# lfalive/fast-genomic-data-processing

Measured on AMD Instinct MI355X. Metric: PairHMM GCUPS, higher is better.
Workload: dtype f32

## Files before the change

### fast-genomic-data-processing_amd/csrc/mgx_pairhmm.hip

```cpp
#include <hip/hip_runtime.h>

#include <algorithm>
#include <atomic>
#include <cerrno>
#include <cmath>
#include <cstdio>
#include <cstdlib>
#include <cstring>
#include <chrono>
#include <memory>
#include <mutex>
#include <new>
#include <thread>
#include <string>
#include <vector>

#include "../../include/mgx_pairhmm.h"
#include "../../include/mgx_realign.h"
#include "mgx_hip_util.h"
#include "mgx_realign_internal.h"
#include "mgx_tables.h"
#include "pairhmm_pack.h"
#include "pairhmm_plan.h"
#include "pairhmm_wire.h"
// ... 463 lines not shown
int ensure_strip_scratch(mgx_pairhmm* c, size_t bytes) {
    if (bytes <= c->strip_cap) return 0;
    HIP_TRY(hipStreamSynchronize(c->compute));
    (void)hipFree(c->d_strip); c->d_strip = nullptr; c->strip_cap = 0;
    HIP_TRY(hipMalloc(&c->d_strip, bytes));
    c->strip_cap = bytes;
    return 0;
}

int pick_event_set(Run& r) {
    mgx_pairhmm_batch* b = r.b;
    if (!r.timing) return 0;
    if (b->ev.empty()) {
        const size_t per = b->bins.size() * 4;
        b->ev_sets = (uint32_t)std::max<size_t>(1, std::min<size_t>(kMaxEventSets, 1024 / per));
        b->ev.resize(per * b->ev_sets);
        for (auto& e : b->ev) HIP_TRY(hipEventCreate(&e));
    }
    r.ev = b->ev.data() + (size_t)(b->runs_timed % b->ev_sets) * b->bins.size() * 4;
    return 0;
}

int begin_run(Run& r) {
    mgx_pairhmm* c = r.c; mgx_pairhmm_batch* b = r.b;
    if (b->uploaded) HIP_TRY(hipStreamWaitEvent(r.s, b->uploaded, 0));
    HIP_TRY(hipMemsetAsync(b->counters(), 0, kCounters * sizeof(uint32_t), r.s));
    HIP_TRY(hipMemsetAsync(b->dev(b->lay.o_used), 0, b->n_pairs, r.s));
    KernelArgs& base = r.base;
    base.jobs = b->dev<Job>(b->lay.jobs);
    base.bases = b->dev(b->lay.seq[kSeqBases]); base.qual = b->dev(b->lay.seq[kSeqQual]); base.ins = b->dev(b->lay.seq[kSeqIns]); base.del = b->dev(b->lay.seq[kSeqDel]);
    base.gcp = b->dev(b->lay.seq[kSeqGcp]); base.hap_bases = b->dev(b->lay.seq[kSeqHap]);
    base.out_log10 = b->dev<double>(b->lay.o_out); base.used_f64 = b->dev(b->lay.o_used);
    base.nhap_list = b->dev<uint32_t>(b->lay.nlist); base.nhap_count = b->counters() + kNhapCount;
    base.log10_initial_f = c->log10_initial_f;
    base.log10_initial_d = c->log10_initial_d;
    return 0;
}

int launch_f64(const Run& r, KernelArgs a, int Gd, int RPLd, uint32_t grid, uint32_t block, uint32_t lds) {
    const mgx_pairhmm* c = r.c;
    a.ph2pr = c->d_ph2pr_d; a.mm = c->d_mm_d; a.ph2pr_div3 = c->d_div3_d; a.gap_ratio = c->d_ratio_d;
    a.rerun_list = r.b->rerun_list() + r.b->n_pairs; a.rerun_count = r.b->counters() + kExactCount;
    KernelFn f = a.strip_scratch ? (KernelFn)pairhmm_fwd_strip<double> : pick_kernel<double>(Gd, RPLd);
    if (!f) { set_error("no fp64 kernel for G=%d RPL=%d", Gd, RPLd); return -ENOSYS; }
    hipLaunchKernelGGL(f, dim3(grid), dim3(block), lds, r.s, a);
    return 0;
}

int launch_multi(Run& r, int gset, const MultiSet& ms) {
    mgx_pairhmm* c = r.c; mgx_pairhmm_batch* b = r.b;
    const std::vector<size_t>& set = ms.members;
    MultiArgs m{};
    m.a = r.base;
    m.a.rerun_list = b->rerun_list(); m.a.rerun_count = b->counters() + kSharedCount;
    m.a.job_list = nullptr; m.a.n_dyn = nullptr;
    m.a.ph2pr = c->d_ph2pr_f; m.a.mm = c->d_mm_f; m.a.ph2pr_div3 = c->d_div3_f; m.a.gap_ratio = c->d_ratio_f;
    m.n_bins = (uint32_t)set.size();
    size_t book = set[0];
    uint64_t cells = 0, bytes = 0;
    for (size_t q = 0; q < set.size(); ++q) {
        const Bin& bn = b->bins[set[q]];
        m.job_first[q] = bn.job_begin; m.job_count[q] = bn.job_count; m.lds_stride[q] = bn.lds_stride;
        m.G[q] = (uint8_t)bn.G; m.RPL[q] = (uint8_t)bn.RPL; m.bin[q] = (uint8_t)set[q];
        if (bn.cells > b->bins[book].cells) book = set[q];
        cells += bn.cells; bytes += bn.alg_bytes;
        r.in_multi[set[q]] = 1;
// ... 144 lines not shown

int mgx_pairhmm_batch_read_inputs(mgx_pairhmm_t* c, mgx_pairhmm_batch_t* b, uint8_t* bases, uint8_t* qual, uint8_t* ins,
                                  uint8_t* del, uint8_t* gcp, uint8_t* hap) {
    if (!c || !b) { set_error("ctx/batch is NULL"); return -EINVAL; }
    if ((b->lay.read_bytes && (!bases || !qual || !ins || !del || !gcp)) || (b->lay.hap_bytes && !hap)) { set_error("NULL argument"); return -EINVAL; }
    HIP_TRY(hipSetDevice(c->device));
    if (b->n_pairs == 0) return 0;
    if (b->uploaded) HIP_TRY(hipEventSynchronize(b->uploaded));
    uint8_t* const host[kSeqArrays] = {bases, qual, ins, del, gcp, hap};
    for (int k = 0; k < kSeqArrays; ++k) {
        const uint64_t len = k == kSeqHap ? b->lay.hap_bytes : b->lay.read_bytes;
        if (len) HIP_TRY(hipMemcpy(host[k], b->dev(b->lay.seq[k]), len, hipMemcpyDeviceToHost));
    }
    return 0;
}

int mgx_pairhmm_sync(mgx_pairhmm_t* c) {
    if (!c) { set_error("ctx is NULL"); return -EINVAL; }
    HIP_TRY(hipSetDevice(c->device));
    HIP_TRY(hipStreamSynchronize(c->compute));
    return 0;
}

int mgx_pairhmm_batch_stats(mgx_pairhmm_t* c, mgx_pairhmm_batch_t* b, mgx_pairhmm_stats_t* out) {
    if (!c || !b || !out) { set_error("NULL argument"); return -EINVAL; }
    HIP_TRY(hipSetDevice(c->device));
    HIP_TRY(hipStreamSynchronize(c->compute));
    mgx_pairhmm_stats_t st = b->stats;
    const bool force_f64 = (c->flags & MGX_PAIRHMM_FORCE_DOUBLE) != 0;
    st.n_launches_f32 = force_f64 ? 0 : (uint32_t)b->bins.size();
    st.n_launches_f64 = (uint32_t)b->bins.size();
    st.n_rerun_f64 = 0;
    st.n_nhap_f32 = 0;
    if (b->ran && b->n_pairs) {
        std::vector<uint32_t> cnt(kCounters);
        HIP_TRY(hipMemcpy(cnt.data(), b->counters(), kCounters * sizeof(uint32_t), hipMemcpyDeviceToHost));
        for (size_t k = 0; k < b->bins.size(); ++k) st.n_nhap_f32 += cnt[kNhapCount + k];
        for (size_t k = 0; k < b->bins.size(); ++k) st.n_rerun_f64 += force_f64 ? b->bins[k].job_count : cnt[k];
        if (!force_f64) st.n_rerun_f64 += cnt[kSharedCount];
        st.n_exact = cnt[kExactCount];
    }
    st.ms_f32 = st.ms_f64 = st.ms_f32_dominant = 0;
    st.dominant_cells = st.dominant_alg_bytes = 0;
    st.dominant_kernel[0] = 0;
    st.n_runs_timed = 0;
    if ((c->flags & MGX_PAIRHMM_TIMING) && b->ran && !b->ev.empty() && b->runs_timed) {
        const uint32_t n_sets = std::min(b->runs_timed, b->ev_sets);
        const bool acct = b->acct_cells.size() == b->bins.size();
        auto cells_of = [&](size_t k) { return acct ? b->acct_cells[k] : b->bins[k].cells; };
        size_t dom = 0;
        for (size_t k = 0; k < b->bins.size(); ++k) if (cells_of(k) >= cells_of(dom)) dom = k;
        double f32 = 0, f64 = 0, domms = 0;
        for (uint32_t q = 0; q < n_sets; ++q) {
            const uint32_t set = (b->runs_timed - 1 - q) % b->ev_sets;
            hipEvent_t* ev = b->ev.data() + (size_t)set * b->bins.size() * 4;
            for (size_t k = 0; k < b->bins.size(); ++k) {
                float ms = 0;
                if (!force_f64) {
                    HIP_TRY(hipEventElapsedTime(&ms, ev[4 * k + 0], ev[4 * k + 1]));
                    f32 += ms;
                    if (k == dom) domms += ms;
                }
                float ms2 = 0;
                HIP_TRY(hipEventElapsedTime(&ms2, ev[4 * k + 2], ev[4 * k + 3]));
                f64 += ms2;
            }
        }
        st.n_runs_timed = n_sets;
        st.ms_f32 = (float)(f32 / n_sets); st.ms_f64 = (float)(f64 / n_sets);
        if (!force_f64) {
// ... 404 lines not shown
```

### fast-genomic-data-processing_amd/csrc/pairhmm_kernels.hip.inc

```

#include <type_traits>

#include "best_allele_rule.h"
#include "pairhmm_plan.h"

namespace {

using namespace mgx_hmm_plan;

struct KernelArgs {
    const Job* jobs;
    const uint32_t* job_list;
    const uint32_t* n_dyn;
    uint32_t n_static;
    uint32_t job_first;
    const uint8_t* bases;
    const uint8_t* qual;
    const uint8_t* ins;
    const uint8_t* del;
    const uint8_t* gcp;
    const uint8_t* hap_bases;
    const void* ph2pr;
    const void* mm;
    const void* ph2pr_div3;
    const void* gap_ratio;
    double* out_log10;
    uint8_t* used_f64;
    uint32_t* rerun_list;
    uint32_t* rerun_count;
    uint32_t* nhap_list;
    uint32_t* nhap_count;
    uint32_t lds_stride;
    void* strip_scratch;
    uint32_t strip_stride;
    float log10_initial_f;
    double log10_initial_d;
};

constexpr double kExactBelow = 1e-280;
constexpr int kCodeN = 4;
constexpr int kCodePad = 7;

__device__ __forceinline__ int base_code(int b) {
    int c = 0;
    c = (b == 'C') ? 1 : c;
    c = (b == 'T') ? 2 : c;
    c = (b == 'G') ? 3 : c;
    c = (b == 'N') ? kCodeN : c;
    return c;
}

__device__ __forceinline__ uint32_t base_code4(uint32_t w) {
    const uint32_t sel = (w >> 1) & 0x07070707u;
    const uint32_t code = __builtin_amdgcn_perm(0x04000000u, 0x03020100u, sel);
    const uint32_t want = __builtin_amdgcn_perm(0x4E000000u, 0x47544341u, sel);
    const uint32_t diff = want ^ w;
    const uint32_t nz = (((diff & 0x7F7F7F7Fu) + 0x7F7F7F7Fu) | diff) & 0x80808080u;
    const uint32_t ok = ((nz ^ 0x80808080u) >> 7) * 0xFFu;
    return code & ok;
}

template <int G> constexpr int lane_stride() { return G < 16 ? 16 / G : 1; }

template <int G>
// ... 7 lines not shown
__device__ __forceinline__ float shr1(float old, float v) {
    return __builtin_bit_cast(float, dpp_shr1<G>(__builtin_bit_cast(int, old), __builtin_bit_cast(int, v)));
}
template <int G>
__device__ __forceinline__ double shr1(double old, double v) {
    long long o = __builtin_bit_cast(long long, old), x = __builtin_bit_cast(long long, v);
    unsigned lo = (unsigned)dpp_shr1<G>((int)(unsigned)o, (int)(unsigned)x);
    unsigned hi = (unsigned)dpp_shr1<G>((int)(unsigned)(o >> 32), (int)(unsigned)(x >> 32));
    return __builtin_bit_cast(double, ((long long)hi << 32) | (long long)lo);
}

template <int G, typename T>
__device__ __forceinline__ T shr1_down(T v) {
    const int lane = (int)(threadIdx.x & 63);
    constexpr int S = lane_stride<G>();
    const int j = G < 16 ? (lane & 15) / S : lane % G;
    const int src = (j == G - 1) ? lane : lane + S;
    return __shfl(v, src, 64);
}

__device__ __forceinline__ float fma_(float a, float b, float c) { return __builtin_fmaf(a, b, c); }
__device__ __forceinline__ double fma_(double a, double b, double c) { return __builtin_fma(a, b, c); }

template <typename T> struct Prec;
template <> struct Prec<float> {
    static __device__ __forceinline__ float initial() { return 0x1p120f; }
};
template <> struct Prec<double> {
    static __device__ __forceinline__ double initial() { return 0x1p1020; }
};

template <int RPL, int CODES> constexpr int etab_bytes_per_wave() { return ((RPL + 1) / 2) * CODES * 64 * 8; }

template <typename T, int G, int RPL, bool STRIP = false, bool EXACT = false, int CODES = kMaxCodes>
__device__ __forceinline__ void pairhmm_body(const KernelArgs& a, uint8_t* smem, const uint32_t block, const uint32_t n_blocks) {
    constexpr int GPW = 64 / G;
    constexpr bool kETab = (sizeof(T) == 4);
    constexpr int kNumCodes = CODES;
    static_assert(CODES == 4 || CODES == kMaxCodes, "four or five code columns");
    static_assert(kETab || CODES == kMaxCodes, "fp64 has no table: the N code is compared");
    constexpr bool kSix = (sizeof(T) == 4) && !EXACT;
    constexpr int RP2 = (RPL + 1) / 2;
    constexpr int S = lane_stride<G>();
    const int gpb = (int)blockDim.x / G;
    const int tid = (int)threadIdx.x;
    const int lane = tid & 63;
    const int wave = tid >> 6;
    const int j = G < 16 ? (lane & 15) / S : lane % G;
    const int grp = wave * GPW + (G < 16 ? (lane >> 4) * S + (lane & 15) % S : lane / G);
    const int n_waves = (int)blockDim.x >> 6;
    uint8_t* etab = smem + (kETab ? (size_t)wave * etab_bytes_per_wave<RPL, CODES>() : 0);
    uint8_t* hapbuf = smem + (kETab ? (size_t)n_waves * etab_bytes_per_wave<RPL, CODES>() : 0) +
                      (size_t)grp * a.lds_stride;
    const T* __restrict__ ph2pr = (const T*)a.ph2pr;
    const T* __restrict__ mm = (const T*)a.mm;
    const T* __restrict__ ph2pr_div3 = (const T*)a.ph2pr_div3;
    const T* __restrict__ gap_ratio = (const T*)a.gap_ratio;
    const uint32_t n_jobs = a.n_dyn ? *a.n_dyn : a.n_static;

    for (uint32_t base = block * (uint32_t)gpb; base < n_jobs; base += n_blocks * (uint32_t)gpb) {
        const uint32_t slot = base + (uint32_t)grp;
        const bool live = slot < n_jobs;
        uint32_t job_idx = 0;
        Job job;
        job.read_off = 0; job.hap_off = 0; job.R = 0; job.H = 0; job.pair = 0; job.pad_ = 0;
        if (live) {
            job_idx = a.job_list ? a.job_list[slot] : a.job_first + slot;
            job = a.jobs[job_idx];
        }
        const int R = (int)job.R, H = (int)job.H;
        constexpr int kStripRows = G * RPL;
        const int n_strips = STRIP ? (R > kStripRows ? (R + kStripRows - 1) / kStripRows : 1) : 1;
        const int first_rows = R - (n_strips - 1) * kStripRows;

        __syncthreads();
        bool hap_n = false;
        {
            const uint8_t* hp = a.hap_bases + job.hap_off;
            const int n_words = (int)a.lds_stride >> 2;
            uint32_t* hb32 = reinterpret_cast<uint32_t*>(hapbuf);
            for (int w = j; w < n_words; w += G) {
                const int c0 = 4 * w - G;
                uint32_t packed;
                if (live && c0 >= 0 && c0 + 4 <= H) {
                    uint32_t raw;
                    __builtin_memcpy(&raw, hp + c0, 4);
                    packed = base_code4(raw);
                } else {
                    packed = 0;
#pragma unroll
                    for (int t = 0; t < 4; ++t) {
                        const int c = c0 + t;
                        const int code = (live && c >= 0 && c < H) ? base_code(hp[c]) : (kNumCodes > 4 ? kCodeN : 0);
                        packed |= (uint32_t)code << (8 * t);
                    }
                }
                if constexpr (kETab && kNumCodes == 4) {
                    const uint32_t x = packed ^ (0x01010101u * (uint32_t)kCodeN);
                    hap_n |= ((x - 0x01010101u) & ~x & 0x80808080u) != 0;
                    packed &= 0x03030303u;
                }
                hb32[w] = packed;
            }
        }
        bool group_hap_n = false;
        if constexpr (kETab && kNumCodes == 4) {
            uint64_t gmask;
            if constexpr (G == 64) gmask = ~0ull;
            else if constexpr (G == 16) gmask = 0xFFFFull << (lane & 48);
            else gmask = (uint64_t)((G == 8 ? 0x5555u : 0x1111u) << ((lane & 15) % S)) << (lane & 48);
            group_hap_n = (__ballot((int)hap_n) & gmask) != 0;
        }

        T sumM = 0, sumX = 0;
        bool zero_gap = false;
        if constexpr (STRIP) {
            for (int rr = lane; rr < R; rr += 64) zero_gap |= (a.gcp[job.read_off + (uint64_t)rr] & 127) == 0;
        }
        int nl = 0;
        T* const bnd = STRIP ? reinterpret_cast<T*>(a.strip_scratch) + (size_t)block * 6u * a.strip_stride : nullptr;
      for (int strip = 0; strip < n_strips; ++strip) {
        const int rows_here = (STRIP && strip > 0) ? kStripRows : first_rows;
        const int row_base = (STRIP && strip > 0) ? first_rows + (strip - 1) * kStripRows : 0;
        const bool last_strip = strip == n_strips - 1;
        nl = (rows_here + RPL - 1) / RPL;
        const int top_clones = nl * RPL - rows_here;
        volatile T* const bcur = STRIP ? bnd + (size_t)(strip & 1) * 3u * a.strip_stride : nullptr;
        const volatile T* const bprev = STRIP ? bnd + (size_t)((strip & 1) ^ 1) * 3u * a.strip_stride : nullptr;
        if (STRIP && strip > 0) __syncthreads();

        T k0[RPL], k1[RPL], k2[RPL], k3[RPL], k4[RPL], eM[RPL], eX[RPL];
        int rb[RPL];
        T pm[RPL], px[RPL], py[RPL];
        bool clone[RPL];
        T ratio[RPL];
        const T init_y = Prec<T>::initial() / (T)(H > 0 ? H : 1);
#pragma unroll
        for (int s = 0; s < RPL; ++s) {
            const int rho = j * RPL + s - top_clones;
            k0[s] = 0; k1[s] = 0; k2[s] = 0; k3[s] = 0; k4[s] = 0; eM[s] = 0; eX[s] = 0;
            rb[s] = 0; pm[s] = 0; px[s] = 0; py[s] = 0; clone[s] = false; ratio[s] = 0;
            if (live && j < nl) {
                if (rho < 0) {
                    clone[s] = true;
                    k3[s] = 1;
                    py[s] = init_y;
                } else {
                    const uint64_t o = job.read_off + (uint64_t)(row_base + rho);
                    const int qi = a.ins[o] & 127, qd = a.del[o] & 127, qc = a.gcp[o] & 127;
                    const int qq = a.qual[o] & 127;
                    const int mn = qi <= qd ? qi : qd, mx = qi <= qd ? qd : qi;
                    k0[s] = mm[((mx * (mx + 1)) >> 1) + mn];
                    k3[s] = ph2pr[qc];
                    k1[s] = (T)1.0 - ph2pr[qc];
                    k2[s] = ph2pr[qi];
                    k4[s] = ph2pr[qd];
                    zero_gap |= (qc == 0);
                    const T distm = ph2pr[qq];
                    eM[s] = (T)1.0 - distm;
                    const int code = base_code(a.bases[o]);
                    eX[s] = (code == kCodeN) ? eM[s] : ph2pr_div3[qq];
                    ratio[s] = gap_ratio[qc];
                    rb[s] = code;
                }
            }
        }
        if constexpr (kETab) {
            float* et = reinterpret_cast<float*>(etab) + lane * 2;
#pragma unroll
            for (int s = 0; s < RPL; ++s)
#pragma unroll
                for (int code = 0; code < kNumCodes; ++code)
                    et[((s >> 1) * kNumCodes + code) * 128 + (s & 1)] =
                        (code == rb[s] || code == kCodeN) ? eM[s] : eX[s];
        }
        __syncthreads();

        const bool swept = live && !group_hap_n;
        const int nsteps_g = swept ? (H + nl - 1) : 0;
        int nmax = nsteps_g, nmin = swept ? nsteps_g : 0x7fffffff;
        if constexpr (GPW > 1) {
#pragma unroll
            for (int off = 1; off < 64; off <<= 1) {
                if (off >= S && off < (G < 16 ? 16 : G)) continue;
                const int o1 = __shfl_xor(nmax, off, 64), o2 = __shfl_xor(nmin, off, 64);
                nmax = o1 > nmax ? o1 : nmax;
                nmin = o2 < nmin ? o2 : nmin;
            }
        }
        nmax = __builtin_amdgcn_readfirstlane(nmax);
        nmin = __builtin_amdgcn_readfirstlane(nmin);
        if (nmin > nmax) nmin = nmax;

        const uint8_t* hp_lane = hapbuf + (G - j);
        const uint8_t* et_lane = etab + lane * 8;

        auto load_e = [&](int h, T (&dst)[RPL]) {
            if constexpr (kETab) {
                const uint8_t* p = et_lane + (h << 9);
#pragma unroll
                for (int s2 = 0; s2 < RP2; ++s2) {
                    const float2 v = *reinterpret_cast<const float2*>(p + s2 * kNumCodes * 512);
                    dst[2 * s2] = v.x;
                    if (2 * s2 + 1 < RPL) dst[2 * s2 + 1] = v.y;
                }
            } else {
                const bool hN = (h == kCodeN);
#pragma unroll
                for (int s = 0; s < RPL; ++s) dst[s] = ((h == rb[s]) | hN) ? eM[s] : eX[s];
            }
        };

        const bool use_plain = EXACT || __any((int)zero_gap) != 0;
        constexpr int kPlain = 0, kScaled = 1, kSixOp = 2;

        auto sweep = [&](auto form_tag) {
            constexpr int FORM = decltype(form_tag)::value;
            constexpr bool SC = FORM == kScaled;
            constexpr bool SIX = FORM == kSixOp;
            T y_above = init_y;
            if constexpr (SC || SIX) {
                T g_own[RPL], g_below[RPL];
#pragma unroll
                for (int s = 0; s < RPL; ++s) g_own[s] = k1[s];
                T g_next_lane = shr1_down<G>(g_own[0]);
#pragma unroll
                for (int s = 0; s < RPL; ++s) g_below[s] = (s + 1 < RPL) ? g_own[s + 1] : g_next_lane;
                if (j == nl - 1) {
                    g_below[RPL - 1] = (T)1.0;
                    if constexpr (STRIP) { if (!last_strip) g_below[RPL - 1] = (T)1.0 - ph2pr[a.gcp[job.read_off + (uint64_t)(row_base + rows_here)] & 127]; }
                }
                T my_above[RPL];
                if constexpr (SIX) {
                    T my_own[RPL];
#pragma unroll
                    for (int s = 0; s < RPL; ++s) my_own[s] = clone[s] ? (T)1.0 : k4[s];
                    T my_top = (T)1.0;
                    if constexpr (STRIP) {
                        if (strip > 0) my_top = ph2pr[a.del[job.read_off + (uint64_t)(row_base - 1)] & 127];
                    }
                    my_above[0] = shr1<G>(my_top, my_own[RPL - 1]);
#pragma unroll
                    for (int s = 1; s < RPL; ++s) my_above[s] = my_own[s - 1];
                }
#pragma unroll
                for (int s = 0; s < RPL; ++s) {
                    if (clone[s]) {
                        py[s] = SIX ? init_y : g_below[s] * init_y;
                    } else {
                        const T gb = g_below[s];
                        const T pMX = k2[s], pXX = k3[s], pMY = k4[s];
                        k1[s] = gb * pMX;
                        k2[s] = gb * ratio[s];
                        if constexpr (SIX) k3[s] = g_own[s] * my_above[s];
                        else k3[s] = gb * pMY;
                        k4[s] = pXX;
                    }
                    if (clone[s]) { k1[s] = 0; k2[s] = 0; k3[s] = 0; k4[s] = 1; }
                }
                y_above = SIX ? init_y : g_own[0] * init_y;
            }
            const T old_y = (j == 0) ? y_above : (T)0;
            T uaM = 0, uaX = 0, uaY = old_y, ubM = 0, ubX = 0, ubY = old_y;
            if constexpr (STRIP) {
                if (strip > 0) {
                    uaY = 0; ubY = 0;
                    if (j == 0 && H > 0) { ubM = bprev[0]; ubX = bprev[a.strip_stride]; ubY = bprev[2u * a.strip_stride]; }
                }
            }

            auto column = [&](const T (&ec)[RPL], T& o2M, T& o2X, T& o2Y, const T o1M, const T o1X, bool count, const int dcol) {
                T Mn[RPL], Xn[RPL], Yn[RPL];
                if constexpr (SIX) {
#pragma unroll
                    for (int s = RPL - 1; s >= 0; --s) {
                        const T t = s ? fma_(k3[s], py[s - 1], fma_(pm[s - 1], k0[s], px[s - 1]))
                                      : fma_(k3[0], o2Y, fma_(o2M, k0[0], o2X));
                        py[s] = fma_(py[s], k4[s], pm[s]);
                        pm[s] = t * ec[s];
                    }
                    px[0] = fma_(o1X, k2[0], o1M * k1[0]);
#pragma unroll
                    for (int s = 1; s < RPL; ++s) px[s] = fma_(px[s - 1], k2[s], pm[s - 1] * k1[s]);
#pragma unroll
                    for (int s = 0; s < RPL; ++s) { Mn[s] = pm[s]; Xn[s] = px[s]; Yn[s] = py[s]; }
                } else if constexpr (SC) {
                    Mn[0] = (fma_(o2M, k0[0], o2X) + o2Y) * ec[0];
                    Xn[0] = fma_(o1X, k2[0], o1M * k1[0]);
                    Yn[0] = fma_(py[0], k4[0], pm[0] * k3[0]);
#pragma unroll
                    for (int s = 1; s < RPL; ++s) {
                        Mn[s] = (fma_(pm[s - 1], k0[s], px[s - 1]) + py[s - 1]) * ec[s];
                        Xn[s] = fma_(Xn[s - 1], k2[s], Mn[s - 1] * k1[s]);
                        Yn[s] = fma_(py[s], k4[s], pm[s] * k3[s]);
                    }
                } else if constexpr (EXACT) {
                    Mn[0] = ((o2M * k0[0] + o2X * k1[0]) + o2Y * k1[0]) * ec[0];
                    Xn[0] = o1M * k2[0] + o1X * k3[0];
                    Yn[0] = pm[0] * k4[0] + py[0] * k3[0];
#pragma unroll
                    for (int s = 1; s < RPL; ++s) {
                        Mn[s] = ((pm[s - 1] * k0[s] + px[s - 1] * k1[s]) + py[s - 1] * k1[s]) * ec[s];
                        Xn[s] = Mn[s - 1] * k2[s] + Xn[s - 1] * k3[s];
                        Yn[s] = pm[s] * k4[s] + py[s] * k3[s];
                    }
                } else {
                    Mn[0] = fma_(o2Y, k1[0], fma_(o2X, k1[0], o2M * k0[0])) * ec[0];
                    Xn[0] = fma_(o1X, k3[0], o1M * k2[0]);
                    Yn[0] = fma_(py[0], k3[0], pm[0] * k4[0]);
#pragma unroll
                    for (int s = 1; s < RPL; ++s) {
                        Mn[s] = fma_(py[s - 1], k1[s], fma_(px[s - 1], k1[s], pm[s - 1] * k0[s])) * ec[s];
                        Xn[s] = fma_(Xn[s - 1], k3[s], Mn[s - 1] * k2[s]);
                        Yn[s] = fma_(py[s], k3[s], pm[s] * k4[s]);
                    }
                }
// ... 9 lines not shown
                        const bool in = c1 < H;
                        o2M = in ? bprev[c1] : (T)0; o2X = in ? bprev[a.strip_stride + c1] : (T)0; o2Y = in ? bprev[2u * a.strip_stride + c1] : (T)0;
                    }
                    if (!last_strip && j == nl - 1) {
                        const int c = dcol - j;
                        if (c >= 0 && c < H) { bcur[c] = Mn[RPL - 1]; bcur[a.strip_stride + c] = Xn[RPL - 1]; bcur[2u * a.strip_stride + c] = Yn[RPL - 1]; }
                    }
                }
            };

            T e[RPL];
            int d = 0;
            int h1 = hp_lane[1];
            load_e((int)hp_lane[0], e);
            for (; d + 2 <= nmin; d += 2) {
                T e1[RPL];
                load_e(h1, e1);
                const int h2 = hp_lane[d + 2], h3 = hp_lane[d + 3];
                column(e, uaM, uaX, uaY, ubM, ubX, true, d);
                load_e(h2, e);
                column(e1, ubM, ubX, ubY, uaM, uaX, true, d + 1);
                h1 = h3;
            }
            for (; d < nmax; ++d) {
                const int hn = hp_lane[d + 1];
                column(e, uaM, uaX, uaY, ubM, ubX, d < nsteps_g, d);
                T t;
                t = uaM; uaM = ubM; ubM = t;
                t = uaX; uaX = ubX; ubX = t;
                t = uaY; uaY = ubY; ubY = t;
                load_e(hn, e);
            }
        };
        if constexpr (EXACT) sweep(std::integral_constant<int, kPlain>{});
        else if (use_plain) sweep(std::integral_constant<int, kPlain>{});
        else if constexpr (kSix) sweep(std::integral_constant<int, kSixOp>{});
        else sweep(std::integral_constant<int, kScaled>{});
      }

        if (live && j == nl - 1) {
            const T res = sumM + sumX;
            if constexpr (sizeof(T) == 4) {
                if (group_hap_n) {
                    const uint32_t k = atomicAdd(a.nhap_count, 1u);
                    a.nhap_list[k] = job_idx;
                } else if (res < 1e-28f) {
                    const uint32_t k = atomicAdd(a.rerun_count, 1u);
                    a.rerun_list[k] = job_idx;
                } else {
                    a.out_log10[job.pair] = (double)(log10f(res) - a.log10_initial_f);
                }
            } else {
                if (!EXACT && a.rerun_count && res < kExactBelow) {
                    const uint32_t k = atomicAdd(a.rerun_count, 1u);
                    a.rerun_list[k] = job_idx;
                } else {
                    a.out_log10[job.pair] = log10(res) - a.log10_initial_d;
                    a.used_f64[job.pair] = 1;
                }
            }
        }
    }
}

template <typename T, int G, int RPL, int CODES = kMaxCodes>
#ifndef MGX_HMM_MINWAVES_8
#define MGX_HMM_MINWAVES_8 4
#endif
__global__ __launch_bounds__(256, (sizeof(T) == 4 && RPL == 7) ? MGX_HMM_MINWAVES_8 : (sizeof(T) == 4 && RPL == 10) ? 3 : 1) void pairhmm_fwd(KernelArgs a) {
    extern __shared__ __attribute__((aligned(16))) uint8_t smem[];
    pairhmm_body<T, G, RPL, false, false, CODES>(a, smem, blockIdx.x, gridDim.x);
}

constexpr int kStripG = 64, kStripRPL = 16;
template <typename T>
__global__ __launch_bounds__(64) void pairhmm_fwd_strip(KernelArgs a) {
    extern __shared__ __attribute__((aligned(16))) uint8_t smem[];
    pairhmm_body<T, kStripG, kStripRPL, true>(a, smem, blockIdx.x, gridDim.x);
}
__global__ __launch_bounds__(64) void pairhmm_fwd_exact(KernelArgs a) {
    extern __shared__ __attribute__((aligned(16))) uint8_t smem[];
    pairhmm_body<double, kStripG, kStripRPL, true, true>(a, smem, blockIdx.x, gridDim.x);
}

struct MultiArgs {
    KernelArgs a;
    uint32_t n_bins;
    uint32_t block_first[kMultiBins + 1];
    uint32_t job_first[kMultiBins], job_count[kMultiBins], lds_stride[kMultiBins];
    uint8_t G[kMultiBins], RPL[kMultiBins];
    uint8_t bin[kMultiBins];
};

template <int GSET>
__device__ __forceinline__ void pairhmm_multi_body(const MultiArgs& m, uint8_t* smem) {
    uint32_t k = 0;
    while (k + 1 < m.n_bins && blockIdx.x >= m.block_first[k + 1]) ++k;
    KernelArgs a = m.a;
    a.job_first = m.job_first[k]; a.n_static = m.job_count[k]; a.lds_stride = m.lds_stride[k];
    a.nhap_list += m.job_first[k]; a.nhap_count += m.bin[k];
    const uint32_t blk = blockIdx.x - m.block_first[k], nblk = m.block_first[k + 1] - m.block_first[k];
    const int code = (int)m.G[k] * 16 + (int)m.RPL[k];
#define MGX_MCASE(g, r) case (g) * 16 + (r): pairhmm_body<float, g, r, false, false, 4>(a, smem, blk, nblk); break;
    if constexpr (GSET == 0) {
        switch (code) {
            MGX_MCASE(16, 1) MGX_MCASE(16, 2) MGX_MCASE(16, 3) MGX_MCASE(16, 4) MGX_MCASE(16, 5) MGX_MCASE(16, 6) MGX_MCASE(16, 7) MGX_MCASE(16, 8)
            default: break;
        }
    } else {
        switch (code) {
            MGX_MCASE(8, 1) MGX_MCASE(8, 2) MGX_MCASE(8, 3) MGX_MCASE(8, 4) MGX_MCASE(8, 5) MGX_MCASE(8, 6) MGX_MCASE(8, 7) MGX_MCASE(8, 8)
            MGX_MCASE(4, 1) MGX_MCASE(4, 2) MGX_MCASE(4, 3) MGX_MCASE(4, 4) MGX_MCASE(4, 5) MGX_MCASE(4, 6) MGX_MCASE(4, 7) MGX_MCASE(4, 8)
            default: break;
        }
    }
#undef MGX_MCASE
}

template <int GSET>
__global__ __launch_bounds__(256) void pairhmm_fwd_multi(MultiArgs m) {
    extern __shared__ __attribute__((aligned(16))) uint8_t smem[];
    pairhmm_multi_body<GSET>(m, smem);
}

__global__ __launch_bounds__(256) void pairhmm_make_jobs_multi(const SeqRef* __restrict__ reads, const uint32_t* __restrict__ read_region,
                                                               const uint32_t* __restrict__ job_prefix, uint32_t n_reads,
                                                               const RegionRef* __restrict__ regions, const SeqRef* __restrict__ haps,
                                                               uint32_t n_jobs, Job* __restrict__ jobs) {
    const uint32_t q = blockIdx.x * 256 + threadIdx.x;
    if (q >= n_jobs) return;
    uint32_t lo = 0, hi = n_reads;
    while (hi - lo > 1) { const uint32_t m = lo + (hi - lo) / 2; if (job_prefix[m] <= q) lo = m; else hi = m; }
    const SeqRef r = reads[lo];
    const RegionRef g = regions[read_region[lo]];
    const SeqRef h = haps[g.hap_begin + (q - job_prefix[lo])];
    Job j;
// ... 108 lines not shown
}
__device__ __forceinline__ mgx_best_allele::Cand shfl_xor_(mgx_best_allele::Cand c, int off) {
    return mgx_best_allele::Cand{__shfl_xor(c.pri, off, 64), (uint32_t)__shfl_xor((int)c.at, off, 64), (uint32_t)__shfl_xor((int)c.entered, off, 64)};
}
__global__ __launch_bounds__(256) void pairhmm_best_allele_rows(const double* __restrict__ values, const uint32_t* __restrict__ row_off,
                                                                const uint32_t* __restrict__ row_nh, const double* __restrict__ priority,
                                                                const uint32_t* __restrict__ pri_off, uint32_t n_rows, int32_t* __restrict__ out_best) {
    namespace BA = mgx_best_allele;
    const uint32_t r = blockIdx.x * 4 + (threadIdx.x >> 6);
    const uint32_t lane = threadIdx.x & 63;
    if (r >= n_rows) return;
    const uint32_t n_haps = row_nh[r];
    const double* row = values + row_off[r];
    BA::Top top = BA::top_identity();
    for (uint32_t h = lane; h < n_haps; h += 64) top = BA::merge(top, BA::top_of(row[h], h));
#pragma unroll
    for (int off = 32; off > 0; off >>= 1) top = BA::merge(top, shfl_xor_(top, off));
    uint32_t best = top.at == BA::kNone ? 0u : top.at;
    if (priority && n_haps > 1) {
        const double* pri = priority + (pri_off ? pri_off[r] : row_off[r]);
        BA::Cand cand = BA::cand_identity();
        for (uint32_t h = lane; h < n_haps; h += 64) cand = BA::merge(cand, BA::cand_of(top, BA::top_of(row[h], h).v, pri[h], h));
#pragma unroll
        for (int off = 32; off > 0; off >>= 1) cand = BA::merge(cand, shfl_xor_(cand, off));
        best = BA::result(top, pri[top.at], cand);
    }
    if (lane == 0) out_best[r] = (int32_t)best;
}

using KernelFn = void (*)(KernelArgs);

template <typename T, int CODES = kMaxCodes>
KernelFn pick_kernel(int G, int RPL) {
#define MGX_CASE(g, r) if (G == g && RPL == r) return pairhmm_fwd<T, g, r, CODES>;
    MGX_CASE(4, 1) MGX_CASE(4, 2) MGX_CASE(4, 3) MGX_CASE(4, 4) MGX_CASE(4, 5) MGX_CASE(4, 6) MGX_CASE(4, 7) MGX_CASE(4, 8)
    MGX_CASE(8, 1) MGX_CASE(8, 2) MGX_CASE(8, 3) MGX_CASE(8, 4) MGX_CASE(8, 5) MGX_CASE(8, 6) MGX_CASE(8, 7) MGX_CASE(8, 8)
    MGX_CASE(16, 1) MGX_CASE(16, 2) MGX_CASE(16, 3) MGX_CASE(16, 4)
    MGX_CASE(16, 5) MGX_CASE(16, 6) MGX_CASE(16, 7) MGX_CASE(16, 8)
    if constexpr (sizeof(T) == 4) { MGX_CASE(16, 9) MGX_CASE(16, 10) MGX_CASE(16, 11) MGX_CASE(16, 12) }
    if constexpr (sizeof(T) == 8) { MGX_CASE(64, 3) }
    MGX_CASE(64, 4) MGX_CASE(64, 5) MGX_CASE(64, 6) MGX_CASE(64, 7) MGX_CASE(64, 8)
    MGX_CASE(64, 9) MGX_CASE(64, 10) MGX_CASE(64, 11) MGX_CASE(64, 12)
    MGX_CASE(64, 13) MGX_CASE(64, 14) MGX_CASE(64, 15) MGX_CASE(64, 16)
#undef MGX_CASE
    return nullptr;
}

}
```

### fast-genomic-data-processing_amd/csrc/pairhmm_plan.h

```cpp
#pragma once

#include <algorithm>
#include <cerrno>
#include <cstdint>
#include <cstring>
#include <vector>

#include "../../include/mgx_pairhmm.h"
#include "mgx_common.h"
#include "pairhmm_wire.h"

#pragma GCC visibility push(hidden)
namespace mgx_hmm_plan {


struct Job {
    uint64_t read_off;
    uint64_t hap_off;
    uint32_t R;
    uint32_t H;
    uint32_t pair;
    uint32_t pad_;
};
static_assert(sizeof(Job) == 32, "Job is 32 bytes");
// ... 42 lines not shown
    bool strip = false;
};

inline void shape_of(uint32_t R, int min_g, int* G, int* RPL) {
    if (R <= (uint32_t)kMaxRowsG4 && min_g <= 4) { *G = 4; *RPL = (int)((R + 3) / 4); }
    else if (R <= (uint32_t)kMaxRowsG8 && min_g <= 8) { *G = 8; *RPL = (int)((R + 7) / 8); }
    else if (R <= (uint32_t)kMaxRowsG16) { *G = 16; *RPL = (int)((R + 15) / 16); }
    else if (R <= (uint32_t)kMaxRowsG64) { *G = 64; *RPL = std::max(kG64MinRPL, (int)((R + 63) / 64)); }
    else if (R <= (uint32_t)kMaxRowsStrip) { *G = 64; *RPL = kStripMarkRPL; }
    else { *G = 0; *RPL = 0; }
}
inline uint32_t hap_stride(uint32_t max_h, int G) { return (max_h + 2u * (uint32_t)G + 8u + 15u) & ~15u; }
inline uint32_t lds_bytes(const Bin& bin, bool f32, int codes = kMaxCodes) {
    const uint32_t waves = bin.block / 64u, groups = bin.block / (uint32_t)(f32 ? bin.G : bin.Gd);
    const uint32_t etab = f32 ? (uint32_t)((bin.RPL + 1) / 2) * (uint32_t)codes * 512u : 0u;
    return waves * etab + groups * bin.lds_stride;
}
constexpr int kBinG8 = kNarrowMaxRPL, kBinG16 = kBinG8 + kG8MaxRPL, kBinG64 = kBinG16 + kG16MaxRPL;
constexpr int kBinStrip = kBinG64 + (kG64MaxRPL - kG64MinRPL + 1);
constexpr int kBins = kBinStrip + 1;
inline int bin_index(int G, int RPL) {
    if (G == 64 && RPL == kStripMarkRPL) return kBinStrip;
    return G == 4 ? RPL - 1 : G == 8 ? kBinG8 + RPL - 1 : G == 16 ? kBinG16 + RPL - 1 : kBinG64 + RPL - kG64MinRPL;
}
inline void bin_shape(int k, Bin* b) {
    if (k == kBinStrip) { b->G = 64; b->RPL = kG64MaxRPL; b->Gd = 64; b->RPLd = kG64MaxRPL; b->strip = true; return; }
    if (k < kBinG8) { b->G = 4; b->RPL = k + 1; }
    else if (k < kBinG16) { b->G = 8; b->RPL = k - kBinG8 + 1; }
    else if (k < kBinG64) { b->G = 16; b->RPL = k - kBinG16 + 1; }
    else { b->G = 64; b->RPL = k - kBinG64 + kG64MinRPL; }
    if (b->G == 16 && b->RPL > 8) { b->Gd = 64; b->RPLd = (16 * b->RPL + 63) / 64; }
    else { b->Gd = b->G; b->RPLd = b->RPL; }
}
constexpr int kExactCount = 62, kSharedCount = 63, kNhapCount = 64, kCounters = 128;
static_assert(kBins <= kExactCount && kNhapCount + kBins <= kCounters, "counter slots");

inline int finalize_bin(Bin& bin, int n_cu, uint32_t block) {
    bin.lds_stride = hap_stride(bin.max_h, std::max(bin.G, bin.Gd));
    bin.block = block;
    while (bin.block > 64u && lds_bytes(bin, true) > kMaxLdsPerBlock) bin.block /= 2;
    if (lds_bytes(bin, true) > kMaxLdsPerLaunch) {
        set_error("haplotype of %u bases does not fit the LDS staging buffer", bin.max_h);
        return -E2BIG;
    }
    if (bin.strip) {
        bin.block = 64;
        bin.grid_f32 = bin.grid_f64 = bin.grid_f64_all = std::min<uint32_t>(bin.job_count, (uint32_t)n_cu * 4u);
        return 0;
    }
    const uint32_t gpb = bin.block / bin.G, gpbd = bin.block / bin.Gd;
    bin.grid_f32 = (bin.job_count + gpb - 1) / gpb;
    bin.grid_f64_all = (bin.job_count + gpbd - 1) / gpbd;
    bin.grid_f64 = std::min<uint32_t>(bin.grid_f64_all, (uint32_t)n_cu * 8u);
    bin.grid_nhap = std::min<uint32_t>(bin.grid_f32, (uint32_t)n_cu * 8u);
    return 0;
}
inline void merge_small_bins(uint64_t (&count)[kBins], int (&remap)[kBins]) {
    for (int k = 0; k < kBins; ++k) remap[k] = k;
    for (int k = 0; k + 1 < kBins; ++k) {
        if (k + 1 == kBinG8 || k + 1 == kBinG16 || k + 1 == kBinG64 || k + 1 == kBinStrip) continue;
        if (count[k] && count[k] < kMergeBelow) { count[k + 1] += count[k]; count[k] = 0; remap[k] = k + 1; }
    }
    for (int k = 0; k < kBins; ++k) { int t = k; while (remap[t] != t) t = remap[t]; remap[k] = t; }
}

inline uint64_t pair_cells(uint64_t R, uint64_t H) { return R * H; }
inline uint64_t pair_bytes(uint64_t R, uint64_t H) { return 5 * R + H + 4; }

// ... 320 lines not shown
```

### fast-genomic-data-processing_amd/native.py

```python
import ctypes as C
import os

_HERE = os.path.dirname(os.path.abspath(__file__))
_LIB = None


class MgxError(RuntimeError):
    pass


def lib_path():
    return os.path.join(_HERE, "libmgx.so")


class PairHMMInput(C.Structure):
    _fields_ = [
        ("n_reads", C.c_uint64), ("read_off", C.c_void_p), ("bases", C.c_void_p),
        ("qual", C.c_void_p), ("ins", C.c_void_p), ("del_", C.c_void_p), ("gcp", C.c_void_p),
        ("n_haps", C.c_uint64), ("hap_off", C.c_void_p), ("hap_bases", C.c_void_p),
        ("n_pairs", C.c_uint64), ("pair_read", C.c_void_p), ("pair_hap", C.c_void_p),
    ]


class PairHMMWire(C.Structure):
    _fields_ = [
        ("n_reads", C.c_uint64), ("n_haps", C.c_uint64), ("n_pairs", C.c_uint64),
        ("read_off", C.c_void_p), ("hap_off", C.c_void_p), ("pair_read", C.c_void_p), ("pair_hap", C.c_void_p),
        ("w_qual", C.c_uint8), ("w_ins", C.c_uint8), ("w_del", C.c_uint8), ("w_gcp", C.c_uint8), ("gcp_const", C.c_uint8),
        ("pad_", C.c_uint8 * 3),
        ("bases4", C.c_void_p), ("qual", C.c_void_p), ("ins", C.c_void_p), ("del_", C.c_void_p), ("gcp", C.c_void_p),
        ("hap4", C.c_void_p),
    ]


class PairHMMStats(C.Structure):
    _fields_ = [
        ("n_pairs", C.c_uint64), ("cells", C.c_uint64), ("alg_bytes", C.c_uint64),
        ("n_rerun_f64", C.c_uint64), ("n_launches_f32", C.c_uint32), ("n_launches_f64", C.c_uint32),
        ("n_runs_timed", C.c_uint32), ("ms_f32", C.c_float), ("ms_f64", C.c_float), ("ms_f32_dominant", C.c_float),
        ("dominant_cells", C.c_uint64), ("dominant_alg_bytes", C.c_uint64),
        ("dominant_kernel", C.c_char * 64), ("n_exact", C.c_uint64),
        ("n_nhap_f32", C.c_uint64),
    ]


class QueueConfig(C.Structure):
    _fields_ = [("n_devices", C.c_uint32), ("devices", C.c_void_p), ("lanes_per_device", C.c_uint32),
                ("depth", C.c_uint32), ("batch_pairs", C.c_uint32), ("flags", C.c_uint)]


class QueueStats(C.Structure):
    _fields_ = [("n_pairs", C.c_uint64), ("n_batches", C.c_uint64), ("cells", C.c_uint64),
                ("bytes_h2d", C.c_uint64), ("bytes_d2h", C.c_uint64), ("seconds", C.c_double),
                ("pack_seconds", C.c_double), ("wait_seconds", C.c_double), ("n_lanes", C.c_uint32),
                ("batches_per_device", C.c_uint64 * 16)]


class ReadModel(C.Structure):
    _fields_ = [("pcr_rate_factor", C.c_int), ("base_quality_threshold", C.c_int), ("constant_gcp", C.c_int),
                ("log10_mismapping_rate", C.c_double), ("max_error_per_base", C.c_double)]


PAIRHMM_SYMBOLS = {
    "mgx_last_error": (C.c_char_p, []),
    "mgx_pairhmm_create": (C.c_int, [C.c_int, C.c_uint, C.POINTER(C.c_void_p)]),
    "mgx_pairhmm_destroy": (None, [C.c_void_p]),
    "mgx_pairhmm_compute": (C.c_int, [C.c_void_p, C.POINTER(PairHMMInput), C.c_void_p]),
    "mgx_pairhmm_compute_regions": (C.c_int, [C.c_void_p, C.c_uint32, C.c_void_p, C.c_void_p]),
    "mgx_pairhmm_batch_create": (C.c_int, [C.c_void_p, C.POINTER(PairHMMInput), C.POINTER(C.c_void_p)]),
    "mgx_pairhmm_batch_run": (C.c_int, [C.c_void_p, C.c_void_p]),
    "mgx_pairhmm_batch_results": (C.c_int, [C.c_void_p, C.c_void_p, C.c_void_p, C.c_void_p]),
    "mgx_pairhmm_batch_stats": (C.c_int, [C.c_void_p, C.c_void_p, C.POINTER(PairHMMStats)]),
    "mgx_pairhmm_batch_destroy": (None, [C.c_void_p, C.c_void_p]),
    "mgx_pairhmm_sync": (C.c_int, [C.c_void_p]),
    "mgx_read_model_defaults": (None, [C.c_void_p]),
# ... 301 lines not shown
```

### include/mgx_pairhmm.h

```cpp
#ifndef MGX_PAIRHMM_H
#define MGX_PAIRHMM_H

#include <stddef.h>
#include <stdint.h>

#ifdef __cplusplus
extern "C" {
#endif

typedef struct mgx_pairhmm mgx_pairhmm_t;
typedef struct mgx_pairhmm_batch mgx_pairhmm_batch_t;

#define MGX_PAIRHMM_FORCE_DOUBLE 1u
#define MGX_PAIRHMM_TIMING       2u
#define MGX_PAIRHMM_PACKED_FP32  4u
#define MGX_PAIRHMM_WIRE         8u
#define MGX_CU_PATTERN(p) (((unsigned)(p) & 0xFFu) << 8)
#define MGX_STREAM_HIGH_PRIORITY (1u << 16)

typedef struct mgx_pairhmm_input {
    uint64_t n_reads;
    const uint64_t* read_off;
    const uint8_t* bases;
    const uint8_t* qual;
    const uint8_t* ins;
    const uint8_t* del;
    const uint8_t* gcp;
    uint64_t n_haps;
    const uint64_t* hap_off;
    const uint8_t* hap_bases;
    uint64_t n_pairs;
    const uint32_t* pair_read;
    const uint32_t* pair_hap;
} mgx_pairhmm_input_t;

typedef struct mgx_pairhmm_stats {
    uint64_t n_pairs;
    uint64_t cells;
    uint64_t alg_bytes;
    uint64_t n_rerun_f64;
    uint32_t n_launches_f32;
    uint32_t n_launches_f64;
    uint32_t n_runs_timed;
    float ms_f32;
    float ms_f64;
    float ms_f32_dominant;
    uint64_t dominant_cells;
    uint64_t dominant_alg_bytes;
    char dominant_kernel[64];
    uint64_t n_exact;
    uint64_t n_nhap_f32;
} mgx_pairhmm_stats_t;

const char* mgx_last_error(void);

#define MGX_DEVICE_AUTO (-1)

int mgx_pairhmm_create(int device, unsigned flags, mgx_pairhmm_t** out);
void mgx_pairhmm_destroy(mgx_pairhmm_t* ctx);

int mgx_pairhmm_compute(mgx_pairhmm_t* ctx, const mgx_pairhmm_input_t* in, double* out_log10);

int mgx_pairhmm_compute_regions(mgx_pairhmm_t* ctx, uint32_t n_regions, const mgx_pairhmm_input_t* regions,
                                double* const* out_log10);

int mgx_pairhmm_batch_create(mgx_pairhmm_t* ctx, const mgx_pairhmm_input_t* in,
                             mgx_pairhmm_batch_t** out);
int mgx_pairhmm_batch_run(mgx_pairhmm_t* ctx, mgx_pairhmm_batch_t* batch);
int mgx_pairhmm_batch_results(mgx_pairhmm_t* ctx, mgx_pairhmm_batch_t* batch, double* out_log10,
                              uint8_t* used_f64);
int mgx_pairhmm_batch_stats(mgx_pairhmm_t* ctx, mgx_pairhmm_batch_t* batch,
                            mgx_pairhmm_stats_t* out);
void mgx_pairhmm_batch_destroy(mgx_pairhmm_t* ctx, mgx_pairhmm_batch_t* batch);
int mgx_pairhmm_sync(mgx_pairhmm_t* ctx);

typedef struct mgx_read_model {
    int pcr_rate_factor;
    int base_quality_threshold;
    int constant_gcp;
    double log10_mismapping_rate;
    double max_error_per_base;
} mgx_read_model_t;
void mgx_read_model_defaults(mgx_read_model_t* m);
int mgx_pairhmm_region(mgx_pairhmm_t* ctx, const mgx_pairhmm_input_t* in, const uint8_t* mapq,
// ... 64 lines not shown
```

Baseline: 7039.

## Add five-operation rescaled fp32 cell recurrence for narrow-group PairHMM kernels

Adds a FIVE template path that algebraically rescales the per-row transition coefficients (reciprocals of match probability, products with neighbour gap terms) so the inner M/X/Y cell update needs fewer multiplies per cell. The path is used for fp32 kernels with four base codes and groups of up to 16 lanes, both in the multi-bin launcher and in pick_kernel. Pairs that have zero gap or zero match coefficients, or whose result overflows, are sent to the existing deferred N-hap fallback list, and a new counter tracks them. The cost is extra per-read setup (divisions, shuffles) and possible extra deferrals to the slower path, with the rescaling also changing fp32 rounding behaviour.

New measurement: 7507, median of 6. 1.07x the previous value.

```diff
diff --git a/fast-genomic-data-processing_amd/csrc/mgx_pairhmm.hip b/fast-genomic-data-processing_amd/csrc/mgx_pairhmm.hip
--- a/fast-genomic-data-processing_amd/csrc/mgx_pairhmm.hip
+++ b/fast-genomic-data-processing_amd/csrc/mgx_pairhmm.hip
@@ -519,6 +519,7 @@
     base.gcp = b->dev(b->lay.seq[kSeqGcp]); base.hap_bases = b->dev(b->lay.seq[kSeqHap]);
     base.out_log10 = b->dev<double>(b->lay.o_out); base.used_f64 = b->dev(b->lay.o_used);
     base.nhap_list = b->dev<uint32_t>(b->lay.nlist); base.nhap_count = b->counters() + kNhapCount;
+    base.form_count = b->counters() + kFormDeferCount;
     base.log10_initial_f = c->log10_initial_f;
     base.log10_initial_d = c->log10_initial_d;
     return 0;
@@ -729,10 +730,13 @@
     st.n_launches_f64 = (uint32_t)b->bins.size();
     st.n_rerun_f64 = 0;
     st.n_nhap_f32 = 0;
+    st.n_form_deferred_f32 = 0;
     if (b->ran && b->n_pairs) {
         std::vector<uint32_t> cnt(kCounters);
         HIP_TRY(hipMemcpy(cnt.data(), b->counters(), kCounters * sizeof(uint32_t), hipMemcpyDeviceToHost));
         for (size_t k = 0; k < b->bins.size(); ++k) st.n_nhap_f32 += cnt[kNhapCount + k];
+        st.n_form_deferred_f32 = cnt[kFormDeferCount];
+        st.n_nhap_f32 -= st.n_form_deferred_f32;
         for (size_t k = 0; k < b->bins.size(); ++k) st.n_rerun_f64 += force_f64 ? b->bins[k].job_count : cnt[k];
         if (!force_f64) st.n_rerun_f64 += cnt[kSharedCount];
         st.n_exact = cnt[kExactCount];
diff --git a/fast-genomic-data-processing_amd/csrc/pairhmm_kernels.hip.inc b/fast-genomic-data-processing_amd/csrc/pairhmm_kernels.hip.inc
--- a/fast-genomic-data-processing_amd/csrc/pairhmm_kernels.hip.inc
+++ b/fast-genomic-data-processing_amd/csrc/pairhmm_kernels.hip.inc
@@ -30,6 +30,7 @@
     uint32_t* rerun_count;
     uint32_t* nhap_list;
     uint32_t* nhap_count;
+    uint32_t* form_count;
     uint32_t lds_stride;
     void* strip_scratch;
     uint32_t strip_stride;
@@ -103,13 +104,14 @@
 
 template <int RPL, int CODES> constexpr int etab_bytes_per_wave() { return ((RPL + 1) / 2) * CODES * 64 * 8; }
 
-template <typename T, int G, int RPL, bool STRIP = false, bool EXACT = false, int CODES = kMaxCodes>
+template <typename T, int G, int RPL, bool STRIP = false, bool EXACT = false, int CODES = kMaxCodes, bool FIVE = false>
 __device__ __forceinline__ void pairhmm_body(const KernelArgs& a, uint8_t* smem, const uint32_t block, const uint32_t n_blocks) {
     constexpr int GPW = 64 / G;
     constexpr bool kETab = (sizeof(T) == 4);
     constexpr int kNumCodes = CODES;
     static_assert(CODES == 4 || CODES == kMaxCodes, "four or five code columns");
     static_assert(kETab || CODES == kMaxCodes, "fp64 has no table: the N code is compared");
+    static_assert(!FIVE || (kETab && CODES == 4 && G <= 16 && !STRIP && !EXACT), "the five-operation cell: first fp32 launch of the classes of up to 16 lanes");
     constexpr bool kSix = (sizeof(T) == 4) && !EXACT;
     constexpr int RP2 = (RPL + 1) / 2;
     constexpr int S = lane_stride<G>();
@@ -175,16 +177,16 @@
             }
         }
         bool group_hap_n = false;
-        if constexpr (kETab && kNumCodes == 4) {
-            uint64_t gmask;
-            if constexpr (G == 64) gmask = ~0ull;
-            else if constexpr (G == 16) gmask = 0xFFFFull << (lane & 48);
-            else gmask = (uint64_t)((G == 8 ? 0x5555u : 0x1111u) << ((lane & 15) % S)) << (lane & 48);
-            group_hap_n = (__ballot((int)hap_n) & gmask) != 0;
-        }
+        uint64_t gmask = ~0ull;
+        if constexpr (G == 16) gmask = 0xFFFFull << (lane & 48);
+        else if constexpr (G < 16) gmask = (uint64_t)((G == 8 ? 0x5555u : 0x1111u) << ((lane & 15) % S)) << (lane & 48);
+        if constexpr (kETab && kNumCodes == 4) group_hap_n = (__ballot((int)hap_n) & gmask) != 0;
 
         T sumM = 0, sumX = 0;
         bool zero_gap = false;
+        bool zero_mm = false;
+        bool defer = group_hap_n;
+        T res_scale = 1;
         if constexpr (STRIP) {
             for (int rr = lane; rr < R; rr += 64) zero_gap |= (a.gcp[job.read_off + (uint64_t)rr] & 127) == 0;
         }
@@ -227,6 +229,7 @@
                     k2[s] = ph2pr[qi];
                     k4[s] = ph2pr[qd];
                     zero_gap |= (qc == 0);
+                    if constexpr (FIVE) zero_mm |= (k0[s] == (T)0);
                     const T distm = ph2pr[qq];
                     eM[s] = (T)1.0 - distm;
                     const int code = base_code(a.bases[o]);
@@ -236,6 +239,39 @@
                 }
             }
         }
+        if constexpr (FIVE) {
+            defer |= (__ballot((int)(zero_gap | zero_mm)) & gmask) != 0;
+            const bool last_lane = j == nl - 1;
+            const T g_next_lane = shr1_down<G>(k1[0]), mm_next_lane = shr1_down<G>(k0[0]);
+            T rcp[RPL], Ap[RPL], gr[RPL];
+#pragma unroll
+            for (int s = 0; s < RPL; ++s) {
+                const T gb = (s + 1 < RPL) ? k1[s + 1] : (last_lane ? (T)1.0 : g_next_lane);
+                const T sb = (s + 1 < RPL) ? k0[s + 1] : (last_lane ? (T)1.0 : mm_next_lane);
+                rcp[s] = (T)1.0 / k0[s];
+                Ap[s] = clone[s] ? (T)0 : (gb * k2[s]) * rcp[s];
+                gr[s] = gb * ratio[s];
+                eM[s] *= sb; eX[s] *= sb;
+            }
+            const T my_up = shr1<G>((T)1.0, clone[RPL - 1] ? (T)1.0 : k4[RPL - 1]);
+            const T a_up = shr1<G>((T)0, Ap[RPL - 1]);
+            T qv[RPL], av[RPL], bv[RPL];
+#pragma unroll
+            for (int s = 0; s < RPL; ++s) {
+                const int rho = j * RPL + s - top_clones;
+                const T my_above = s ? (clone[s - 1] ? (T)1.0 : k4[s - 1]) : my_up;
+                av[s] = s ? Ap[s - 1] : a_up;
+                qv[s] = rho == 0 ? k1[s] : (k1[s] * my_above) * rcp[s];
+                bv[s] = (gr[s] * av[s]) / Ap[s];
+            }
+#pragma unroll
+            for (int s = 0; s < RPL; ++s) {
+                k4[s] = k3[s];
+                k1[s] = av[s]; k2[s] = bv[s]; k3[s] = qv[s];
+                if (clone[s]) { k1[s] = 0; k2[s] = 0; k3[s] = 0; k4[s] = 1; }
+            }
+            res_scale = Ap[RPL - 1];
+        }
         if constexpr (kETab) {
             float* et = reinterpret_cast<float*>(etab) + lane * 2;
 #pragma unroll
@@ -247,7 +283,7 @@
         }
         __syncthreads();
 
-        const bool swept = live && !group_hap_n;
+        const bool swept = live && !defer;
         const int nsteps_g = swept ? (H + nl - 1) : 0;
         int nmax = nsteps_g, nmin = swept ? nsteps_g : 0x7fffffff;
         if constexpr (GPW > 1) {
@@ -283,12 +319,13 @@
         };
 
         const bool use_plain = EXACT || __any((int)zero_gap) != 0;
-        constexpr int kPlain = 0, kScaled = 1, kSixOp = 2;
+        constexpr int kPlain = 0, kScaled = 1, kSixOp = 2, kFiveOp = 3;
 
         auto sweep = [&](auto form_tag) {
             constexpr int FORM = decltype(form_tag)::value;
             constexpr bool SC = FORM == kScaled;
             constexpr bool SIX = FORM == kSixOp;
+            constexpr bool FIV = FORM == kFiveOp;
             T y_above = init_y;
             if constexpr (SC || SIX) {
                 T g_own[RPL], g_below[RPL];
@@ -353,6 +390,19 @@
                     px[0] = fma_(o1X, k2[0], o1M * k1[0]);
 #pragma unroll
                     for (int s = 1; s < RPL; ++s) px[s] = fma_(px[s - 1], k2[s], pm[s - 1] * k1[s]);
+#pragma unroll
+                    for (int s = 0; s < RPL; ++s) { Mn[s] = pm[s]; Xn[s] = px[s]; Yn[s] = py[s]; }
+                } else if constexpr (FIV) {
+#pragma unroll
+                    for (int s = RPL - 1; s >= 0; --s) {
+                        const T t = s ? fma_(k3[s], py[s - 1], fma_(k1[s], px[s - 1], pm[s - 1]))
+                                      : fma_(k3[0], o2Y, fma_(k1[0], o2X, o2M));
+                        py[s] = fma_(py[s], k4[s], pm[s]);
+                        pm[s] = t * ec[s];
+                    }
+                    px[0] = fma_(o1X, k2[0], o1M);
+#pragma unroll
+                    for (int s = 1; s < RPL; ++s) px[s] = fma_(px[s - 1], k2[s], pm[s - 1]);
 #pragma unroll
                     for (int s = 0; s < RPL; ++s) { Mn[s] = pm[s]; Xn[s] = px[s]; Yn[s] = py[s]; }
                 } else if constexpr (SC) {
@@ -428,18 +478,20 @@
                 load_e(hn, e);
             }
         };
-        if constexpr (EXACT) sweep(std::integral_constant<int, kPlain>{});
+        if constexpr (FIVE) sweep(std::integral_constant<int, kFiveOp>{});
+        else if constexpr (EXACT) sweep(std::integral_constant<int, kPlain>{});
         else if (use_plain) sweep(std::integral_constant<int, kPlain>{});
         else if constexpr (kSix) sweep(std::integral_constant<int, kSixOp>{});
         else sweep(std::integral_constant<int, kScaled>{});
       }
 
         if (live && j == nl - 1) {
-            const T res = sumM + sumX;
+            const T res = FIVE ? sumM + res_scale * sumX : sumM + sumX;
             if constexpr (sizeof(T) == 4) {
-                if (group_hap_n) {
+                if (defer || (FIVE && !(res <= 3.402823466e+38f))) {
                     const uint32_t k = atomicAdd(a.nhap_count, 1u);
                     a.nhap_list[k] = job_idx;
+                    if constexpr (FIVE) { if (!group_hap_n) atomicAdd(a.form_count, 1u); }
                 } else if (res < 1e-28f) {
                     const uint32_t k = atomicAdd(a.rerun_count, 1u);
                     a.rerun_list[k] = job_idx;
@@ -459,13 +511,13 @@
     }
 }
 
-template <typename T, int G, int RPL, int CODES = kMaxCodes>
+template <typename T, int G, int RPL, int CODES = kMaxCodes, bool FIVE = false>
 #ifndef MGX_HMM_MINWAVES_8
 #define MGX_HMM_MINWAVES_8 4
 #endif
 __global__ __launch_bounds__(256, (sizeof(T) == 4 && RPL == 7) ? MGX_HMM_MINWAVES_8 : (sizeof(T) == 4 && RPL == 10) ? 3 : 1) void pairhmm_fwd(KernelArgs a) {
     extern __shared__ __attribute__((aligned(16))) uint8_t smem[];
-    pairhmm_body<T, G, RPL, false, false, CODES>(a, smem, blockIdx.x, gridDim.x);
+    pairhmm_body<T, G, RPL, false, false, CODES, FIVE>(a, smem, blockIdx.x, gridDim.x);
 }
 
 constexpr int kStripG = 64, kStripRPL = 16;
@@ -497,7 +549,7 @@
     a.nhap_list += m.job_first[k]; a.nhap_count += m.bin[k];
     const uint32_t blk = blockIdx.x - m.block_first[k], nblk = m.block_first[k + 1] - m.block_first[k];
     const int code = (int)m.G[k] * 16 + (int)m.RPL[k];
-#define MGX_MCASE(g, r) case (g) * 16 + (r): pairhmm_body<float, g, r, false, false, 4>(a, smem, blk, nblk); break;
+#define MGX_MCASE(g, r) case (g) * 16 + (r): pairhmm_body<float, g, r, false, false, 4, true>(a, smem, blk, nblk); break;
     if constexpr (GSET == 0) {
         switch (code) {
             MGX_MCASE(16, 1) MGX_MCASE(16, 2) MGX_MCASE(16, 3) MGX_MCASE(16, 4) MGX_MCASE(16, 5) MGX_MCASE(16, 6) MGX_MCASE(16, 7) MGX_MCASE(16, 8)
@@ -672,7 +724,7 @@
 
 template <typename T, int CODES = kMaxCodes>
 KernelFn pick_kernel(int G, int RPL) {
-#define MGX_CASE(g, r) if (G == g && RPL == r) return pairhmm_fwd<T, g, r, CODES>;
+#define MGX_CASE(g, r) if (G == g && RPL == r) return pairhmm_fwd<T, g, r, CODES, (CODES == 4 && g <= 16)>;
     MGX_CASE(4, 1) MGX_CASE(4, 2) MGX_CASE(4, 3) MGX_CASE(4, 4) MGX_CASE(4, 5) MGX_CASE(4, 6) MGX_CASE(4, 7) MGX_CASE(4, 8)
     MGX_CASE(8, 1) MGX_CASE(8, 2) MGX_CASE(8, 3) MGX_CASE(8, 4) MGX_CASE(8, 5) MGX_CASE(8, 6) MGX_CASE(8, 7) MGX_CASE(8, 8)
     MGX_CASE(16, 1) MGX_CASE(16, 2) MGX_CASE(16, 3) MGX_CASE(16, 4)
diff --git a/fast-genomic-data-processing_amd/csrc/pairhmm_plan.h b/fast-genomic-data-processing_amd/csrc/pairhmm_plan.h
--- a/fast-genomic-data-processing_amd/csrc/pairhmm_plan.h
+++ b/fast-genomic-data-processing_amd/csrc/pairhmm_plan.h
@@ -98,8 +98,8 @@
     if (b->G == 16 && b->RPL > 8) { b->Gd = 64; b->RPLd = (16 * b->RPL + 63) / 64; }
     else { b->Gd = b->G; b->RPLd = b->RPL; }
 }
-constexpr int kExactCount = 62, kSharedCount = 63, kNhapCount = 64, kCounters = 128;
-static_assert(kBins <= kExactCount && kNhapCount + kBins <= kCounters, "counter slots");
+constexpr int kFormDeferCount = 61, kExactCount = 62, kSharedCount = 63, kNhapCount = 64, kCounters = 128;
+static_assert(kBins <= kFormDeferCount && kNhapCount + kBins <= kCounters, "counter slots");
 
 inline int finalize_bin(Bin& bin, int n_cu, uint32_t block) {
     bin.lds_stride = hap_stride(bin.max_h, std::max(bin.G, bin.Gd));
diff --git a/fast-genomic-data-processing_amd/native.py b/fast-genomic-data-processing_amd/native.py
--- a/fast-genomic-data-processing_amd/native.py
+++ b/fast-genomic-data-processing_amd/native.py
@@ -40,7 +40,7 @@
         ("n_runs_timed", C.c_uint32), ("ms_f32", C.c_float), ("ms_f64", C.c_float), ("ms_f32_dominant", C.c_float),
         ("dominant_cells", C.c_uint64), ("dominant_alg_bytes", C.c_uint64),
         ("dominant_kernel", C.c_char * 64), ("n_exact", C.c_uint64),
-        ("n_nhap_f32", C.c_uint64),
+        ("n_nhap_f32", C.c_uint64), ("n_form_deferred_f32", C.c_uint64),
     ]
 
 
diff --git a/include/mgx_pairhmm.h b/include/mgx_pairhmm.h
--- a/include/mgx_pairhmm.h
+++ b/include/mgx_pairhmm.h
@@ -50,6 +50,7 @@
     char dominant_kernel[64];
     uint64_t n_exact;
     uint64_t n_nhap_f32;
+    uint64_t n_form_deferred_f32;
 } mgx_pairhmm_stats_t;
 
 const char* mgx_last_error(void);
```
